# oviniciuscesar/Pseudo-Quadrature-Mirror-Filter

Hardware: NVIDIA B200
Metric: PQMF analyze+inverse throughput (n_band=16) (higher is better)
Workload: dtype f32

## Files before the change

pseudo-quadrature-mirror-filter_b200/csrc/experiments/trace_h4.cu:

```cuda
#define PQMF_H4_TRACE 1
#include <cstdio>
#include <vector>
#include "../hankel4.cuh"
using namespace pqmf;
int main(int argc, char** argv) {
  const bool pair = argc > 4 && atoi(argv[4]) != 0;
  const int B = 64; const long T = 1 << 20, F = T / 16;
  float *x, *y; uint16_t* bank; long long* tr;
  cudaMalloc(&x, (size_t)B * T * 4); cudaMalloc(&y, (size_t)B * T * 4); cudaMalloc(&bank, 2 * 27 * 4096); cudaMalloc(&tr, (64 * 64 + 512) * 8);
  cudaMemset(x, 0, (size_t)B * T * 4); cudaMemset(bank, 0, 2 * 27 * 4096); cudaMemset(tr, 0, 64 * 64 * 8);
  if (argc > 1) {
    std::vector<float> hx(1 << 22), hk(16 * 512);
    srand(3);
    for (auto& v : hx) v = (float)rand() / RAND_MAX - 0.5f;
    for (auto& v : hk) v = ((float)rand() / RAND_MAX - 0.5f) * 0.05f;
    for (size_t o = 0; o < (size_t)B * T; o += hx.size()) cudaMemcpy(x + o, hx.data(), hx.size() * 4, cudaMemcpyHostToDevice);
    std::vector<uint16_t> ia(27 * 2048), is(27 * 2048);
    hankel4_build_banks(hk.data(), 16, 512, 64, 384, ia.data(), is.data());
    cudaMemcpy(bank, ia.data(), ia.size() * 2, cudaMemcpyHostToDevice);
  }
  cudaEvent_t e0, e1; cudaEventCreate(&e0); cudaEventCreate(&e1);
  H4AnalysisParams p{};
  p.x = x; p.y = y; p.bank = bank; p.T = T; p.F = F; p.off = 256; p.parity = 0; p.trace = tr; p.trim_lo = p.trim_hi = argc > 3 ? atoi(argv[3]) : 0; p.g = h4_shape(16, 64, 384, pair, false);
  for (int rep = 0; rep < 3; ++rep) {
    int rc = (pair ? h4_launch_analysis<16, true>(p, B, 0) : h4_launch_analysis<16, false>(p, B, 0));
    cudaError_t e = cudaDeviceSynchronize();
    if (rc || e) { printf("launch rc=%d cuda=%s\n", rc, cudaGetErrorString(e)); return 1; }
  }
  const bool synth = argc > 2 && argv[2][0] == 's';
  H4SynthesisParams q{};
  q.s = x; q.out = y; q.bank = bank; q.F = F; q.o = 16; q.parity = 0; q.trace = tr; q.trim_lo = q.trim_hi = argc > 3 ? atoi(argv[3]) : 0; q.g = h4_shape(16, 64, 384, pair, true);
  if (synth) {
    cudaMemset(tr, 0, 64 * 64 * 8);
    (pair ? h4_launch_synthesis<16, true>(q, B, 0) : h4_launch_synthesis<16, false>(q, B, 0));
    cudaError_t e = cudaDeviceSynchronize();
    if (e) { printf("synthesis cuda=%s\n", cudaGetErrorString(e)); return 1; }
  }
  cudaEventRecord(e0);
  for (int rep = 0; rep < 20; ++rep) { if (synth) (pair ? h4_launch_synthesis<16, true>(q, B, 0) : h4_launch_synthesis<16, false>(q, B, 0)); else (pair ? h4_launch_analysis<16, true>(p, B, 0) : h4_launch_analysis<16, false>(p, B, 0)); }
  cudaEventRecord(e1); cudaDeviceSynchronize();
  float ms = 0; cudaEventElapsedTime(&ms, e0, e1);
  printf("%s %s data: %.1f us per launch (20 back to back)\n", synth ? "synthesis" : "analysis", argc > 1 ? "random" : "zero", ms * 50.f);
  std::vector<long long> h(64 * 64 + 512);
  cudaMemcpy(h.data(), tr, h.size() * 8, cudaMemcpyDeviceToHost);
  {
    long long cmin = 1LL << 60, cmax = 0, nmin = 1LL << 60, nmax = 0;
    for (int i = 0; i < 148; ++i) {
      const long long c = h[64 * 64 + 2 * i], n = h[64 * 64 + 2 * i + 1];
      cmin = c < cmin ? c : cmin; cmax = c > cmax ? c : cmax; nmin = n < nmin ? n : nmin; nmax = n > nmax ? n : nmax;
    }
    printf("per-CTA lifetime: %lld..%lld cycles, %lld..%lld ns -> SM clock %.0f MHz (CTA 0: %lld cycles / %lld ns)\n", cmin, cmax, nmin, nmax,
           1e3 * (double)cmax / (double)nmax, h[64 * 64], h[64 * 64 + 1]);
  }
  const long long t00 = h[(0 * 8 + 1) * 8 + 0];
  printf("warp 1 (MMA warp) and warp 5; cycles relative to the first stamp\n");
  printf("it |  start   conv   loads+publish  wait+drain(it-lag) | period\n");
  long long prev = t00;
  for (int it = 0; it < 56; ++it) {
    for (int w : {1, 5}) {
      long long* r = &h[((size_t)it * 8 + w) * 8];
      if (!r[0]) continue;
      printf("%2d w%d %8lld %6lld %6lld %10lld", it, w, r[0] - t00, r[1] - r[0], r[2] - r[1], r[5] - r[2]);
      if (w == 1) { printf(" | %lld", r[0] - prev); prev = r[0]; }
      printf("\n");
    }
    if (it == 12) it = 40;
  }
  return 0;
}
```

pseudo-quadrature-mirror-filter_b200/csrc/hankel4.cuh:

```cuda
#pragma once
#include <cuda_fp16.h>
#include <cuda_runtime.h>
#include <math.h>
#include <stdint.h>
#include <string.h>

#include <atomic>

#include "half_io.cuh"
#include "hankel16.cuh"
#include "pcm.cuh"
#include "ptx.cuh"

namespace pqmf {

constexpr int kH4Workers = 256;
constexpr int kH4Threads = kH4Workers + 32;
constexpr int kH4SynWorkers = 288;
constexpr int kH4SynThreads = kH4SynWorkers + 32;
constexpr int kH4Rows = 128;
constexpr int kH4TileSamples = 64 * kH4Rows;
constexpr int kH4MaxPlaneRows = 144;
constexpr float kH4Res = 2048.0f;

__device__ __forceinline__ uint64_t umma_desc_sw128(uint32_t smem_addr) {
  uint64_t d = 0;
  d |= (uint64_t)((smem_addr & 0x3FFFFu) >> 4);
  d |= (uint64_t)1 << 16;
  d |= (uint64_t)(1024u >> 4) << 32;
  d |= (uint64_t)1 << 46;
  d |= (uint64_t)2 << 61;
  return d;
}
__device__ __forceinline__ uint32_t sw128_offset(uint32_t byte_lin) { return byte_lin ^ (((byte_lin >> 7) & 7u) << 4); }

struct H4Shape {
  int jlo, kt, ks;
  int rows, plane;
  int bank;
  int bytes;
};
inline H4Shape h4_shape(int M, int jlo, int kt, bool pair, bool synthesis, int extra_pad_bytes = 0) {
  H4Shape g;
  g.jlo = jlo;
  g.kt = kt;
  g.ks = (kt + 64 - M + 15) / 16;
  const int pad_bytes = (synthesis ? 3 * 2 * M : 0) + extra_pad_bytes;
  g.rows = kH4Rows + (32 * g.ks + pad_bytes - 1) / 128;
  g.plane = ((g.rows * 128 + 1023) / 1024) * 1024;
  g.bank = g.ks * 2 * (pair ? 96 : 128) * 16;
  g.bytes = g.bank + 4 * g.plane + 128;
  return g;
}
inline bool h4_shape_fits(const H4Shape& g) { return g.rows <= kH4MaxPlaneRows && g.bytes <= 227 * 1024; }

template <bool PAIR>
__device__ __forceinline__ void h4_issue_mmas(uint32_t d_tmem, uint32_t plane1_addr, uint32_t plane2_addr, uint32_t bank_addr, int ks,
                                              int pad_bytes, int tlo, int thi) {
  constexpr uint32_t kBankRows = PAIR ? 96 : 128;
  const uint64_t da1 = umma_desc_sw128(plane1_addr), da2 = umma_desc_sw128(plane2_addr);
  const uint64_t db = ptx::umma_desc(bank_addr, kBankRows * 16, 128);
  const uint64_t db64 = PAIR ? ptx::umma_desc(bank_addr + 64 * 16, kBankRows * 16, 128) : db;
  constexpr uint32_t m = PAIR ? 256 : 128;
  constexpr uint32_t idesc128 = ptx::umma_idesc_f16(m, 128), idesc64 = ptx::umma_idesc_f16(m, 64);
  constexpr uint32_t kStep = 2 * kBankRows;
  auto a_step = [&](int s) {
    const uint32_t byte = 32u * (uint32_t)s + (uint32_t)pad_bytes;
    return (uint64_t)(8u * (byte >> 7) + ((byte >> 4) & 7u));
  };
  auto mma = [&](uint32_t d, uint64_t a, uint64_t bdesc, uint32_t idesc, bool acc) {
    if constexpr (PAIR) ptx::umma_pair_f16(d, a, bdesc, idesc, acc);
    else ptx::umma_f16(d, a, bdesc, idesc, acc);
  };
  for (int s = tlo; s < ks - thi; ++s) mma(d_tmem, da1 + a_step(s), db + (uint64_t)(kStep * s), idesc128, s != tlo);
  for (int s = 0; s < tlo; ++s) mma(d_tmem, da1 + a_step(s), db64 + (uint64_t)(kStep * s), idesc64, true);
  for (int s = ks - thi; s < ks; ++s) mma(d_tmem, da1 + a_step(s), db64 + (uint64_t)(kStep * s), idesc64, true);
  for (int s = tlo; s < ks - thi; ++s) mma(d_tmem + 64u, da2 + a_step(s), db64 + (uint64_t)(kStep * s), idesc64, true);
}

__device__ __forceinline__ void split2_f16s(float a, float b, uint32_t& h1_bits, uint32_t& h2_bits) {
  const __half2 h1 = __floats2half2_rn(a, b);
  const float2 h1f = __half22float2(h1);
  const float2 r = __ffma2_rn(h1f, make_float2(-kH4Res, -kH4Res), __fmul2_rn(make_float2(a, b), make_float2(kH4Res, kH4Res)));
  const __half2 h2 = __floats2half2_rn(r.x, r.y);
  h1_bits = *reinterpret_cast<const uint32_t*>(&h1);
  h2_bits = *reinterpret_cast<const uint32_t*>(&h2);
}
__device__ __forceinline__ float2 h4_combine2(uint32_t d0a, uint32_t d0b, uint32_t d1a, uint32_t d1b) {
  const float2 t = __ffma2_rn(make_float2(__uint_as_float(d1a), __uint_as_float(d1b)), make_float2(1.0f / kH4Res, 1.0f / kH4Res),
                              make_float2(__uint_as_float(d0a), __uint_as_float(d0b)));
  constexpr float kInv = 1.0f / (float)(1 << kH16ScaleLog2);
  return __fmul2_rn(t, make_float2(kInv, kInv));
}

template <int N>
__device__ __forceinline__ void h4_tmem_ld(uint32_t taddr, uint32_t (&r)[N]) {
  static_assert(N == 2 || N == 4 || N == 8 || N == 16 || N == 32, "columns per load");
  if constexpr (N == 2) ptx::tmem_ld2(taddr, r);
  else if constexpr (N == 4) ptx::tmem_ld4(taddr, r);
  else if constexpr (N == 8) ptx::tmem_ld8(taddr, r);
  else if constexpr (N == 16) ptx::tmem_ld16(taddr, r);
  else ptx::tmem_ld32(taddr, r);
}

#ifdef PQMF_H4_TRACE
#define H4_STAMP(k) do { if (blockIdx.x == 0 && (tid & 31) == 0 && it < 64) p.trace[((size_t)it * 8 + warp) * 8 + (k)] = clock64(); } while (0)
#else
#define H4_STAMP(k) do { } while (0)
#endif

struct H4Smem {
  unsigned char *bank, *planes;
  uint64_t *pfull, *mma_bar, *bankfull;
  uint32_t* tmem_slot;
};
__device__ __forceinline__ H4Smem h4_carve(unsigned char* smem, const H4Shape& g) {
  H4Smem s;
  s.bank = smem;
  s.planes = smem + g.bank;
  s.pfull = reinterpret_cast<uint64_t*>(smem + g.bank + 4 * g.plane);
  s.mma_bar = s.pfull + 2;
  s.bankfull = s.mma_bar + 2;
  s.tmem_slot = reinterpret_cast<uint32_t*>(s.bankfull + 1);
  return s;
}

template <bool PAIR>
__device__ __forceinline__ uint32_t h4_prologue(const H4Smem& s, const H4Shape& g, const uint16_t* bank_images, uint32_t rank, int worker_warps,
                                                int tid) {
  const int warp = tid >> 5;
  ptx::grid_dep_launch();
  if (tid == 0) {
    for (int i = 0; i < 2; ++i) {
      ptx::mbar_init(&s.pfull[i], worker_warps * (PAIR ? 2 : 1));
      ptx::mbar_init(&s.mma_bar[i], 1);
    }
    ptx::mbar_init(s.bankfull, 1);
    ptx::fence_barrier_init();
    ptx::mbar_arrive_expect_tx(s.bankfull, (uint32_t)g.bank);
    ptx::bulk_g2s(s.bank, reinterpret_cast<const unsigned char*>(bank_images) + (size_t)rank * g.bank, (uint32_t)g.bank, s.bankfull);
  }
  if (warp == 0) {
    if constexpr (PAIR) {
      ptx::tmem_alloc_pair(s.tmem_slot, 256);
    } else {
      ptx::tmem_alloc(s.tmem_slot, 256);
      ptx::tmem_relinquish();
    }
  }
  ptx::tc_fence_before();
  __syncthreads();
  if constexpr (PAIR) ptx::cluster_sync_all();
  ptx::tc_fence_after();
  ptx::grid_dep_wait();
  return *s.tmem_slot;
}

template <bool PAIR>
__device__ __forceinline__ void h4_teardown(uint32_t tmem, int warp) {
  ptx::tc_fence_before();
  __syncthreads();
  if constexpr (PAIR) {
    ptx::cluster_sync_all();
    if (warp == 0) ptx::tmem_dealloc_pair(tmem, 256);
  } else {
    if (warp == 0) ptx::tmem_dealloc(tmem, 256);
  }
}

template <bool PAIR>
__device__ __forceinline__ void h4_issuer_loop(const H4Smem& s, const H4Shape& g, uint32_t tmem, unsigned n_iter, int pad_bytes, int tlo,
                                               int thi, unsigned it0 = 0) {
  const uint32_t bank_addr = ptx::smem_u32(s.bank), plane_addr = ptx::smem_u32(s.planes);
  for (unsigned it = it0; it < it0 + n_iter; ++it) {
    const int pb = (int)(it & 1);
    ptx::mbar_wait(&s.pfull[pb], (it >> 1) & 1);
    ptx::tc_fence_after();
    if (ptx::elect_one_sync()) {
      h4_issue_mmas<PAIR>(tmem + (uint32_t)(pb * 128), plane_addr + (2 * pb) * g.plane, plane_addr + (2 * pb + 1) * g.plane, bank_addr, g.ks,
                          pad_bytes, tlo, thi);
      if constexpr (PAIR) ptx::umma_pair_commit(&s.mma_bar[pb]);
      else ptx::umma_commit(&s.mma_bar[pb]);
    }
    __syncwarp();
  }
}

template <bool PAIR>
__device__ __forceinline__ void h4_publish(const H4Smem& s, uint32_t pfull_leader, unsigned it, int pb, int tid, unsigned it0 = 0, unsigned bank_phase = 0) {
  ptx::fence_proxy_async();
  ptx::tc_fence_before();
  __syncwarp();
  if ((tid & 31) == 0) {
    if (it == it0) ptx::mbar_wait(s.bankfull, bank_phase & 1);
    if constexpr (PAIR) ptx::mbar_arrive_cluster(pfull_leader + 8u * pb);
    else ptx::mbar_arrive(&s.pfull[pb]);
  }
}

struct H4AnalysisParams {
  const float* x;
  PcmIn in;
  float* y;
  const uint16_t* bank;
  long T, F;
  int off;
  int parity;
  int trim_lo, trim_hi;
  int accumulate;
  int keep_in_l2;
  H4Shape g;
  long tiles_per_row, n_tiles;
#ifdef PQMF_H4_TRACE
  long long* trace;
#endif
};

template <int M, bool PAIR, H4Io IO>
__global__ void __launch_bounds__(kH4Threads, 1) h4_analysis_kernel(H4AnalysisParams p) {
  constexpr bool PCM = IO == H4Io::PCM, HALF = h4_io_half(IO);
  constexpr int FR = 64 / M;
  constexpr int HB = M / 2;
  constexpr int NO = (kH4MaxPlaneRows * 8 + kH4Workers - 1) / kH4Workers;
  extern __shared__ __align__(1024) unsigned char h4_smem[];
  const H4Shape g = p.g;
  const H4Smem sm = h4_carve(h4_smem, g);
  const int tid = threadIdx.x, warp = tid >> 5;
  constexpr int kMmaWarp = kH4Workers / 32;
  const uint32_t rank = PAIR ? ptx::cluster_ctarank() : 0u;
  const uint32_t tmem = h4_prologue<PAIR>(sm, g, p.bank, rank, kH4Workers / 32, tid);
  const uint32_t pfull_leader = PAIR ? ptx::mapa_shared(ptx::smem_u32(sm.pfull), 0) : 0u;

  const unsigned tpr = (unsigned)p.tiles_per_row;
  const unsigned step_b = gridDim.x / tpr, step_c = gridDim.x % tpr;
  unsigned b = blockIdx.x / tpr, c = blockIdx.x % tpr;
  const unsigned first_tile = PAIR ? (blockIdx.x & ~1u) : blockIdx.x;
  const unsigned n_iter = (unsigned)((p.n_tiles - first_tile + gridDim.x - 1) / gridDim.x);
  const unsigned n_rows = (unsigned)(p.n_tiles / p.tiles_per_row);
#ifdef PQMF_H4_TRACE
  long long cta_c0 = clock64(), cta_t0;
  asm volatile("mov.u64 %0, %%globaltimer;" : "=l"(cta_t0));
#endif

  if (warp == kMmaWarp) {
    if (rank == 0) h4_issuer_loop<PAIR>(sm, g, tmem, n_iter, 0, p.trim_lo, p.trim_hi);
  } else {
    const int n_octs = g.rows * 8;
    float x0[NO][8];
    auto load_window = [&](unsigned bb, unsigned cc) {
      const long s0 = (long)cc * kH4TileSamples + g.jlo - p.off;
      const float* xrow = p.x + (size_t)bb * p.T;
      const uint16_t* xhrow = reinterpret_cast<const uint16_t*>(p.x) + (size_t)bb * p.T;
#pragma unroll
      for (int r = 0; r < NO; ++r) {
        const int o = tid + kH4Workers * r;
        const long s = s0 + 8L * o;
        if (bb < n_rows && o < n_octs && s >= 0 && s < p.T) {
          if constexpr (PCM) {
            pcm_load8_raw(p.in, bb, s, p.T, x0[r]);
          } else if constexpr (HALF) {
            const float4 raw = ptx::ldg128_na(reinterpret_cast<const float4*>(xhrow + s));
            x0[r][0] = raw.x; x0[r][1] = raw.y; x0[r][2] = raw.z; x0[r][3] = raw.w;
          } else {
            ptx::ldg256_na(xrow + s, x0[r]);
          }
        } else {
#pragma unroll
          for (int e = 0; e < 8; ++e) x0[r][e] = 0.f;
        }
      }
    };
    auto convert = [&](int pb, unsigned bb, unsigned cc) {
      unsigned char* p1 = sm.planes + (2 * pb) * g.plane;
      unsigned char* p2 = p1 + g.plane;
#pragma unroll
      for (int r = 0; r < NO; ++r) {
        const int o = tid + kH4Workers * r;
        if (o < n_octs) {
          if constexpr (PCM) {
            const long s = (long)cc * kH4TileSamples + g.jlo - p.off + 8L * o;
            if (bb < n_rows && s >= 0 && s < p.T) pcm_convert8(p.in, bb, x0[r]);
          }
          if constexpr (HALF) h4_widen8<IO>(x0[r]);
          uint4 a, bq;
          split2_f16s(x0[r][0], x0[r][1], a.x, bq.x);
          split2_f16s(x0[r][2], x0[r][3], a.y, bq.y);
          split2_f16s(x0[r][4], x0[r][5], a.z, bq.z);
          split2_f16s(x0[r][6], x0[r][7], a.w, bq.w);
          const uint32_t off = sw128_offset((uint32_t)o * 16u);
          *reinterpret_cast<uint4*>(p1 + off) = a;
          *reinterpret_cast<uint4*>(p2 + off) = bq;
        }
      }
    };
    auto advance = [&](unsigned& bb, unsigned& cc) {
      bb += step_b;
      cc += step_c;
      if (cc >= tpr) {
        cc -= tpr;
        ++bb;
      }
    };
    auto epilogue = [&](unsigned bb, unsigned cc, int dbuf) {
      const int i = tid & 127, hb = tid >> 7;
      const uint32_t taddr = tmem + ((uint32_t)((warp & 3) * 32) << 16) + (uint32_t)(dbuf * 128 + HB * hb);
      const long n = ((long)cc * kH4Rows + i) * FR;
      uint32_t r0[FR][HB], r1[FR][HB];
#pragma unroll
      for (int dl = 0; dl < FR; ++dl) {
        h4_tmem_ld<HB>(taddr + dl * M, r0[dl]);
        h4_tmem_ld<HB>(taddr + 64 + dl * M, r1[dl]);
      }
      ptx::tmem_ld_wait();
      float v[FR][HB];
#pragma unroll
      for (int dl = 0; dl < FR; ++dl) {
        const uint32_t flip = (((FR > 1 ? dl : (int)(n & 1)) + p.parity) & 1) == 0 ? 0x80000000u : 0u;
#pragma unroll
        for (int kk = 0; kk < HB; kk += 2) {
          const float2 t = h4_combine2(r0[dl][kk], r0[dl][kk + 1], r1[dl][kk], r1[dl][kk + 1]);
          v[dl][kk] = t.x;
          v[dl][kk + 1] = __uint_as_float(__float_as_uint(t.y) ^ flip);
        }
      }
      if constexpr (HALF) {
        uint16_t* yp = reinterpret_cast<uint16_t*>(p.y) + ((size_t)bb * M + HB * hb) * p.F + n;
        if (n + FR - 1 < p.F && (p.F % (FR >= 8 ? 8 : FR)) == 0) {
#pragma unroll
          for (int kk = 0; kk < HB; ++kk) {
            uint16_t* q = yp + (size_t)kk * p.F;
            if constexpr (FR >= 8) {
#pragma unroll
              for (int d8 = 0; d8 < FR; d8 += 8) {
                const uint4 w = make_uint4(h4_narrow2<IO>(v[d8][kk], v[d8 + 1][kk]), h4_narrow2<IO>(v[d8 + 2][kk], v[d8 + 3][kk]),
                                           h4_narrow2<IO>(v[d8 + 4][kk], v[d8 + 5][kk]), h4_narrow2<IO>(v[d8 + 6][kk], v[d8 + 7][kk]));
                if (p.keep_in_l2) *reinterpret_cast<uint4*>(q + d8) = w;
                else __stcs(reinterpret_cast<uint4*>(q + d8), w);
              }
            } else if constexpr (FR == 4) {
              const uint2 w = make_uint2(h4_narrow2<IO>(v[0][kk], v[1][kk]), h4_narrow2<IO>(v[2][kk], v[3][kk]));
              if (p.keep_in_l2) *reinterpret_cast<uint2*>(q) = w;
              else __stcs(reinterpret_cast<uint2*>(q), w);
            } else if constexpr (FR == 2) {
              __stcs(reinterpret_cast<unsigned int*>(q), h4_narrow2<IO>(v[0][kk], v[1][kk]));
            } else {
              __stcs(reinterpret_cast<unsigned short*>(q), h4_narrow1<IO>(v[0][kk]));
            }
          }
        } else {
#pragma unroll
          for (int kk = 0; kk < HB; ++kk)
#pragma unroll
            for (int dl = 0; dl < FR; ++dl)
              if (n + dl < p.F) yp[(size_t)kk * p.F + dl] = h4_narrow1<IO>(v[dl][kk]);
        }
        return;
      }
      float* yp = p.y + ((size_t)bb * M + HB * hb) * p.F + n;
      if (n + FR - 1 < p.F && (p.F % (FR >= 4 ? 4 : FR)) == 0) {
        if (p.accumulate) {
          float prev[FR][HB];
#pragma unroll
          for (int kk = 0; kk < HB; ++kk)
#pragma unroll
            for (int dl = 0; dl < FR; ++dl) prev[dl][kk] = __ldcs(yp + (size_t)kk * p.F + dl);
#pragma unroll
          for (int kk = 0; kk < HB; ++kk)
#pragma unroll
            for (int dl = 0; dl < FR; ++dl) v[dl][kk] += prev[dl][kk];
        }
#pragma unroll
        for (int kk = 0; kk < HB; ++kk) {
          float* q = yp + (size_t)kk * p.F;
          if constexpr (FR >= 4) {
#pragma unroll
            for (int d4 = 0; d4 < FR; d4 += 4) {
              const float4 w = make_float4(v[d4][kk], v[d4 + 1][kk], v[d4 + 2][kk], v[d4 + 3][kk]);
              if (p.keep_in_l2) *reinterpret_cast<float4*>(q + d4) = w;
              else __stcs(reinterpret_cast<float4*>(q + d4), w);
            }
          } else if constexpr (FR == 2) {
            __stcs(reinterpret_cast<float2*>(q), make_float2(v[0][kk], v[1][kk]));
          } else {
            __stcs(q, v[0][kk]);
          }
        }
      } else {
#pragma unroll
        for (int kk = 0; kk < HB; ++kk)
#pragma unroll
          for (int dl = 0; dl < FR; ++dl)
            if (n + dl < p.F) yp[(size_t)kk * p.F + dl] = v[dl][kk] + (p.accumulate ? yp[(size_t)kk * p.F + dl] : 0.f);
      }
    };

    unsigned b1 = b, c1 = c;
    advance(b1, c1);
    load_window(b, c);
    unsigned prev_b = 0, prev_c = 0;
    for (unsigned it = 0; it < n_iter; ++it) {
      const int pb = (int)(it & 1);
      H4_STAMP(0);
      convert(pb, b, c);
      H4_STAMP(1);
      h4_publish<PAIR>(sm, pfull_leader, it, pb, tid);
      if (it + 1 < n_iter) load_window(b1, c1);
      H4_STAMP(2);
      if (it > 0) {
        ptx::mbar_wait(&sm.mma_bar[(it - 1) & 1], ((it - 1) >> 1) & 1);
        ptx::tc_fence_after();
        if (prev_b < n_rows) epilogue(prev_b, prev_c, (int)((it - 1) & 1));
      }
      H4_STAMP(5);
      prev_b = b;
      prev_c = c;
      b = b1;
      c = c1;
      advance(b1, c1);
    }
    ptx::mbar_wait(&sm.mma_bar[(n_iter - 1) & 1], ((n_iter - 1) >> 1) & 1);
    ptx::tc_fence_after();
    if (prev_b < n_rows) epilogue(prev_b, prev_c, (int)((n_iter - 1) & 1));
  }
#ifdef PQMF_H4_TRACE
  __syncthreads();
  if (tid == 0) {
    long long t1;
    asm volatile("mov.u64 %0, %%globaltimer;" : "=l"(t1));
    p.trace[64 * 64 + 2 * blockIdx.x] = clock64() - cta_c0;
    p.trace[64 * 64 + 2 * blockIdx.x + 1] = t1 - cta_t0;
  }
#endif
  h4_teardown<PAIR>(tmem, warp);
}

struct H4SynthesisParams {
  const float* s;
  float* out;
  int16_t* pcm_out;
  int C;
  int duo;
  const uint16_t* bank;
  long F;
  int o;
  int parity;
  int trim_lo, trim_hi;
  int accumulate;
  int reverse;
  H4Shape g;
  long tiles_per_row, n_tiles;
#ifdef PQMF_H4_TRACE
  long long* trace;
#endif
};

template <int M, bool PAIR, H4Io IO>
__global__ void __launch_bounds__(kH4SynThreads, 1) h4_synthesis_kernel(H4SynthesisParams p) {
  constexpr bool PCM = IO == H4Io::PCM, HALF = h4_io_half(IO);
  constexpr int FR = 64 / M;
  constexpr int NBG = M >= 8 ? M / 8 : 1;
  constexpr int FPI = M >= 8 ? 4 : 32 / M;
  extern __shared__ __align__(1024) unsigned char h4s_smem[];
  const H4Shape g = p.g;
  const H4Smem sm = h4_carve(h4s_smem, g);
  const int tid = threadIdx.x, warp = tid >> 5;
  constexpr int kMmaWarp = kH4SynWorkers / 32;
  const uint32_t rank = PAIR ? ptx::cluster_ctarank() : 0u;
  const uint32_t tmem = h4_prologue<PAIR>(sm, g, p.bank, rank, kH4SynWorkers / 32, tid);
  const uint32_t pfull_leader = PAIR ? ptx::mapa_shared(ptx::smem_u32(sm.pfull), 0) : 0u;

  const unsigned tpr = (unsigned)p.tiles_per_row;
  const unsigned step_b = gridDim.x / tpr, step_c = gridDim.x % tpr;
  unsigned b = blockIdx.x / tpr, c = blockIdx.x % tpr;
  const unsigned first_tile = PAIR ? (blockIdx.x & ~1u) : blockIdx.x;
  const unsigned G = (PCM && p.duo) ? 2u : 1u;
  const unsigned n_iter = G * (unsigned)((p.n_tiles - first_tile + gridDim.x - 1) / gridDim.x);
  const unsigned n_rows = (unsigned)(p.n_tiles / p.tiles_per_row);

  const int ehi = (g.jlo + g.kt) / M - 1;
  const int pad = (p.o - ehi) & 3;
  const int nbase = p.o - ehi - pad;
  if (warp == kMmaWarp) {
    if (rank == 0) h4_issuer_loop<PAIR>(sm, g, tmem, n_iter, 2 * M * pad, p.trim_lo, p.trim_hi);
  } else {
    const int n_fq = (g.rows * FR + FPI - 1) / FPI;
    const int bg = tid / n_fq, fq = tid - bg * n_fq;
    const bool has_item = tid < n_fq * NBG;
    float4 v0[8];
    auto load4h = [&](const uint16_t* at, bool ok) {
      if (!ok) return make_float4(0.f, 0.f, 0.f, 0.f);
      const float2 raw = ptx::ldg64_na(at);
      return make_float4(raw.x, raw.y, 0.f, 0.f);
    };
    auto load_frames = [&](float4 (&v)[8], unsigned bb, unsigned cc, unsigned hh) {
      if (p.reverse && bb < n_rows) {
        bb = n_rows - 1 - bb;
        cc = tpr - 1 - cc;
      }
      const long n = (long)cc * (kH4Rows * FR) + nbase + FPI * fq;
      const bool live = bb < n_rows && has_item;
      const size_t row = (size_t)bb * G + hh;
      if constexpr (HALF) {
        if constexpr (M >= 8) {
          const uint16_t* sp = reinterpret_cast<const uint16_t*>(p.s) + (row * M + 8 * bg) * p.F + n;
          const bool ok = live && n >= 0 && n + 3 < p.F;
#pragma unroll
          for (int kk = 0; kk < 8; ++kk) v[kk] = load4h(sp + (size_t)kk * p.F, ok);
        } else {
          const uint16_t* sp = reinterpret_cast<const uint16_t*>(p.s) + row * M * p.F + n;
#pragma unroll
          for (int kk = 0; kk < 8; ++kk) {
            const int b4 = kk >> 1, h = kk & 1;
            v[kk] = load4h(sp + (size_t)b4 * p.F + 4 * h, live && n + 4 * h >= 0 && n + 4 * h + 3 < p.F);
          }
        }
      } else if constexpr (M >= 8) {
        const float* sp = p.s + (row * M + 8 * bg) * p.F + n;
        const bool ok = live && n >= 0 && n + 3 < p.F;
#pragma unroll
        for (int kk = 0; kk < 8; ++kk) v[kk] = ok ? ptx::ldg128_na(reinterpret_cast<const float4*>(sp + (size_t)kk * p.F)) : make_float4(0.f, 0.f, 0.f, 0.f);
      } else {
        const float* sp = p.s + row * M * p.F + n;
#pragma unroll
        for (int kk = 0; kk < 8; ++kk) {
          const int b4 = kk >> 1, h = kk & 1;
          const bool ok = live && n + 4 * h >= 0 && n + 4 * h + 3 < p.F;
          v[kk] = ok ? ptx::ldg128_na(reinterpret_cast<const float4*>(sp + (size_t)b4 * p.F + 4 * h)) : make_float4(0.f, 0.f, 0.f, 0.f);
        }
      }
    };
    const uint32_t flip_even = (p.parity & 1) ? 0u : 0x80000000u, flip_odd = flip_even ^ 0x80000000u;
    auto advance = [&](unsigned& bb, unsigned& cc) {
      bb += step_b;
      cc += step_c;
      if (cc >= tpr) {
        cc -= tpr;
        ++bb;
      }
    };
    auto convert = [&](const float4 (&v)[8], int pb) {
      if (!has_item) return;
      unsigned char* p1 = sm.planes + (2 * pb) * g.plane;
      auto comp = [](const float4& q, int c) { return c == 0 ? q.x : c == 1 ? q.y : c == 2 ? q.z : q.w; };
#pragma unroll
      for (int j = 0; j < 4; ++j) {
        float w[8];
        uint32_t o;
        if constexpr (M >= 8) {
          const uint32_t fl = (j & 1) ? flip_odd : flip_even;
#pragma unroll
          for (int kk = 0; kk < 8; ++kk) {
            const float t = comp(v[kk], j);
            w[kk] = (kk & 1) ? __uint_as_float(__float_as_uint(t) ^ fl) : t;
          }
          o = sw128_offset((uint32_t)(4 * fq + j) * (2u * M) + 16u * bg);
        } else {
#pragma unroll
          for (int kk = 0; kk < 8; ++kk) {
            const int b4 = kk & 3, odd = kk >> 2;
            const float t = comp(v[2 * b4 + (j >> 1)], 2 * (j & 1) + odd);
            w[kk] = (b4 & 1) ? __uint_as_float(__float_as_uint(t) ^ (odd ? flip_odd : flip_even)) : t;
          }
          o = sw128_offset((uint32_t)(8 * fq + 2 * j) * (2u * M));
        }
        uint4 h1, h2;
        split2_f16s(w[0], w[1], h1.x, h2.x);
        split2_f16s(w[2], w[3], h1.y, h2.y);
        split2_f16s(w[4], w[5], h1.z, h2.z);
        split2_f16s(w[6], w[7], h1.w, h2.w);
        *reinterpret_cast<uint4*>(p1 + o) = h1;
        *reinterpret_cast<uint4*>(p1 + g.plane + o) = h2;
      }
    };
    uint32_t held[4][4];
    auto epilogue = [&](unsigned bb, unsigned cc, unsigned hh, int dbuf) {
      if (p.reverse) {
        bb = n_rows - 1 - bb;
        cc = tpr - 1 - cc;
      }
      const size_t row = (size_t)bb * G + hh;
      const int i = tid & 127, hb = tid >> 7, lane = tid & 31;
      const uint32_t taddr = tmem + ((uint32_t)((warp & 3) * 32) << 16) + (uint32_t)(dbuf * 128 + 2 * hb * 16);
      uint32_t r0[2][16], r1[2][16];
      ptx::tmem_ld16(taddr, r0[0]);
      ptx::tmem_ld16(taddr + 64, r1[0]);
      ptx::tmem_ld16(taddr + 16, r0[1]);
      ptx::tmem_ld16(taddr + 80, r1[1]);
      ptx::tmem_ld_wait();
      float val[4][8];
#pragma unroll
      for (int q = 0; q < 4; ++q)
#pragma unroll
        for (int e = 0; e < 8; e += 2) {
          const int c0 = 8 * (q & 1) + e;
          const float2 t = h4_combine2(r0[q >> 1][c0], r0[q >> 1][c0 + 1], r1[q >> 1][c0], r1[q >> 1][c0 + 1]);
          val[q][e] = t.x;
          val[q][e + 1] = t.y;
        }
      const bool b0 = lane & 1, b1 = lane & 2;
#pragma unroll
      for (int pr = 0; pr < 2; ++pr)
#pragma unroll
        for (int e = 0; e < 8; ++e) {
          const float recv = __shfl_xor_sync(0xffffffffu, b0 ? val[2 * pr][e] : val[2 * pr + 1][e], 1);
          val[2 * pr + 1][e] = b0 ? val[2 * pr + 1][e] : recv;
          val[2 * pr][e] = b0 ? recv : val[2 * pr][e];
        }
#pragma unroll
      for (int u = 0; u < 2; ++u)
#pragma unroll
        for (int e = 0; e < 8; ++e) {
          const float recv = __shfl_xor_sync(0xffffffffu, b1 ? val[u][e] : val[u + 2][e], 2);
          val[u + 2][e] = b1 ? val[u + 2][e] : recv;
          val[u][e] = b1 ? recv : val[u][e];
        }
      const long total = p.F * M;
      const long t0 = (long)cc * kH4TileSamples + 64 * (i & ~3) + 32 * hb + 8 * (lane & 3);
      if constexpr (PCM) {
        if (G == 2) {
#pragma unroll
          for (int q = 0; q < 4; ++q) {
            uint32_t w[4];
#pragma unroll
            for (int k = 0; k < 4; ++k)
              w[k] = (uint32_t)(uint16_t)pcm_quantise(val[q][2 * k]) | ((uint32_t)(uint16_t)pcm_quantise(val[q][2 * k + 1]) << 16);
            if (hh == 0) {
#pragma unroll
              for (int k = 0; k < 4; ++k) held[q][k] = w[k];
            } else if (t0 + 64 * q + 7 < total) {
              float lr[8];
#pragma unroll
              for (int k = 0; k < 4; ++k) {
                lr[2 * k] = __uint_as_float(__byte_perm(held[q][k], w[k], 0x5410));
                lr[2 * k + 1] = __uint_as_float(__byte_perm(held[q][k], w[k], 0x7632));
              }
              ptx::stg256_cs(reinterpret_cast<float*>(p.pcm_out + ((size_t)bb * total + t0 + 64 * q) * 2), lr);
            }
          }
          return;
        }
#pragma unroll
        for (int q = 0; q < 4; ++q)
          if (t0 + 64 * q + 7 < total) pcm_store8(p.pcm_out, p.C, (long)row, t0 + 64 * q, total, val[q]);
        return;
      }
      if constexpr (HALF) {
        uint16_t* op = reinterpret_cast<uint16_t*>(p.out) + row * total + t0;
#pragma unroll
        for (int q = 0; q < 4; ++q)
          if (t0 + 64 * q + 7 < total) {
            const uint4 w = make_uint4(h4_narrow2<IO>(val[q][0], val[q][1]), h4_narrow2<IO>(val[q][2], val[q][3]), h4_narrow2<IO>(val[q][4], val[q][5]),
                                       h4_narrow2<IO>(val[q][6], val[q][7]));
            __stcs(reinterpret_cast<uint4*>(op + (size_t)q * 64), w);
          }
        return;
      }
      float* op = p.out + row * total + t0;
#pragma unroll
      for (int q = 0; q < 4; ++q)
        if (t0 + 64 * q + 7 < total) {
          if (p.accumulate) {
            float prev[8];
            ptx::ldg256_cs(op + (size_t)q * 64, prev);
#pragma unroll
            for (int e = 0; e < 8; ++e) val[q][e] += prev[e];
          }
          ptx::stg256_cs(op + (size_t)q * 64, val[q]);
        }
    };

    auto next_visit = [&](unsigned& bb, unsigned& cc, unsigned& hh) {
      if (++hh == G) {
        hh = 0;
        advance(bb, cc);
      }
    };
    unsigned h = 0, b1 = b, c1 = c, h1 = 0;
    next_visit(b1, c1, h1);
    load_frames(v0, b, c, h);
    unsigned prev_b = 0, prev_c = 0, prev_h = 0;
    for (unsigned it = 0; it < n_iter; ++it) {
      const int pb = (int)(it & 1);
      H4_STAMP(0);
      if constexpr (HALF) {
        float4 w[8];
#pragma unroll
        for (int kk = 0; kk < 8; ++kk) w[kk] = h4_widen4<IO>(v0[kk]);
        convert(w, pb);
      } else {
        convert(v0, pb);
      }
      H4_STAMP(1);
      h4_publish<PAIR>(sm, pfull_leader, it, pb, tid);
      if (it + 1 < n_iter) load_frames(v0, b1, c1, h1);
      H4_STAMP(2);
      if (it > 0) {
        ptx::mbar_wait(&sm.mma_bar[(it - 1) & 1], ((it - 1) >> 1) & 1);
        ptx::tc_fence_after();
        if (warp < 8 && prev_b < n_rows) epilogue(prev_b, prev_c, prev_h, (int)((it - 1) & 1));
      }
      H4_STAMP(5);
      prev_b = b;
      prev_c = c;
      prev_h = h;
      b = b1;
      c = c1;
      h = h1;
      next_visit(b1, c1, h1);
    }
    ptx::mbar_wait(&sm.mma_bar[(n_iter - 1) & 1], ((n_iter - 1) >> 1) & 1);
    ptx::tc_fence_after();
    if (warp < 8 && prev_b < n_rows) epilogue(prev_b, prev_c, prev_h, (int)((n_iter - 1) & 1));
  }
  h4_teardown<PAIR>(tmem, warp);
}

struct H4Configured {
  std::atomic<int> bytes[64];
  H4Configured() {
    for (auto& b : bytes) b.store(0, std::memory_order_relaxed);
  }
};
inline int h4_sm_count(int dev) {
  static std::atomic<int> sm_count[64];
  int n = sm_count[dev].load(std::memory_order_relaxed);
  if (n == 0) {
    cudaDeviceGetAttribute(&n, cudaDevAttrMultiProcessorCount, dev);
    n = n > 0 ? n : 148;
    sm_count[dev].store(n, std::memory_order_relaxed);
  }
  return n;
}
template <typename Kern>
inline int h4_configure(Kern kern, int bytes, H4Configured& configured, int& sm_count_out) {
  int dev = 0;
  cudaGetDevice(&dev);
  dev &= 63;
  if (configured.bytes[dev].load(std::memory_order_acquire) < bytes) {
    cudaError_t e = cudaFuncSetAttribute(kern, cudaFuncAttributeMaxDynamicSharedMemorySize, bytes);
    if (e != cudaSuccess) return (int)e;
    int seen = configured.bytes[dev].load(std::memory_order_relaxed);
    while (seen < bytes && !configured.bytes[dev].compare_exchange_weak(seen, bytes, std::memory_order_release)) {
    }
  }
  sm_count_out = h4_sm_count(dev);
  return 0;
}

template <bool PAIR, typename Kern, typename Params>
inline int h4_launch(Kern kern, Params p, int B, long row_samples, int threads, H4Configured& configured, cudaStream_t st) {
  int sms = 0;
  if (!h4_shape_fits(p.g)) return -2;
  if (int e = h4_configure(kern, p.g.bytes, configured, sms)) return e;
  p.tiles_per_row = (row_samples + kH4TileSamples - 1) / kH4TileSamples;
  p.n_tiles = p.tiles_per_row * B;
  if (p.tiles_per_row >= (1L << 31) || p.n_tiles >= (1L << 40)) return -2;
  long grid = PAIR ? (sms & ~1) : sms;
  const long want = PAIR ? ((p.n_tiles + 1) & ~1L) : p.n_tiles;
  if (grid > want) grid = want;
  if constexpr (PAIR) {
    cudaLaunchConfig_t cfg = {};
    cfg.gridDim = dim3((unsigned)grid);
    cfg.blockDim = dim3((unsigned)threads);
    cfg.dynamicSmemBytes = (size_t)p.g.bytes;
    cfg.stream = st;
    cudaLaunchAttribute attr[2];
    attr[0].id = cudaLaunchAttributeClusterDimension;
    attr[0].val.clusterDim.x = 2;
    attr[0].val.clusterDim.y = 1;
    attr[0].val.clusterDim.z = 1;
    attr[1].id = cudaLaunchAttributeProgrammaticStreamSerialization;
    attr[1].val.programmaticStreamSerializationAllowed = 1;
    cfg.attrs = attr;
    cfg.numAttrs = 2;
    return (int)cudaLaunchKernelEx(&cfg, kern, p);
  } else {
    kern<<<(unsigned)grid, threads, p.g.bytes, st>>>(p);
    return (int)cudaGetLastError();
  }
}

template <int M, bool PAIR>
int h4_launch_analysis(H4AnalysisParams p, int B, cudaStream_t st, H4Io io = H4Io::F32) {
  static H4Configured configured[4];
  if (p.in.pcm != nullptr) io = H4Io::PCM;
  if (io != H4Io::F32) {
    if constexpr (PAIR) {
      switch (io) {
        case H4Io::PCM: return h4_launch<PAIR>(h4_analysis_kernel<M, PAIR, H4Io::PCM>, p, B, p.F * M, kH4Threads, configured[1], st);
        case H4Io::F16: return h4_launch<PAIR>(h4_analysis_kernel<M, PAIR, H4Io::F16>, p, B, p.F * M, kH4Threads, configured[2], st);
        case H4Io::BF16: return h4_launch<PAIR>(h4_analysis_kernel<M, PAIR, H4Io::BF16>, p, B, p.F * M, kH4Threads, configured[3], st);
        default: return -2;
      }
    } else {
      return -2;
    }
  }
  return h4_launch<PAIR>(h4_analysis_kernel<M, PAIR, H4Io::F32>, p, B, p.F * M, kH4Threads, configured[0], st);
}

template <int M, bool PAIR>
int h4_launch_synthesis(H4SynthesisParams p, int B, cudaStream_t st, H4Io io = H4Io::F32) {
  static H4Configured configured[4];
  if (p.pcm_out != nullptr) {
    if constexpr (PAIR) {
      p.duo = (p.C == 2 && B % 2 == 0) ? 1 : 0;
      return h4_launch<PAIR>(h4_synthesis_kernel<M, PAIR, H4Io::PCM>, p, p.duo ? B / 2 : B, p.F * M, kH4SynThreads, configured[1], st);
    } else {
      return -2;
    }
  }
  if (h4_io_half(io)) {
    if constexpr (PAIR) {
      if (io == H4Io::F16) return h4_launch<PAIR>(h4_synthesis_kernel<M, PAIR, H4Io::F16>, p, B, p.F * M, kH4SynThreads, configured[2], st);
      return h4_launch<PAIR>(h4_synthesis_kernel<M, PAIR, H4Io::BF16>, p, B, p.F * M, kH4SynThreads, configured[3], st);
    } else {
      return -2;
    }
  }
  return h4_launch<PAIR>(h4_synthesis_kernel<M, PAIR, H4Io::F32>, p, B, p.F * M, kH4SynThreads, configured[0], st);
}

inline void hankel4_build_banks(const float* hk , int M, int L, int jlo, int kt, uint16_t* img_analysis, uint16_t* img_synthesis) {
  auto bits = [](float v) {
    const __half h = __float2half_rn(v);
    uint16_t u;
    memcpy(&u, &h, 2);
    return u;
  };
  const int ks = (kt + 64 - M + 15) / 16, kp = 16 * ks;
  const int elo = jlo / M, ehi = (jlo + kt) / M - 1;
  const float sa = (float)(1 << kH16ScaleLog2), ss = (float)M * sa;
  for (int kc = 0; kc < kp / 8; ++kc)
    for (int row = 0; row < 128; ++row)
      for (int e8 = 0; e8 < 8; ++e8) {
        const int kap = 8 * kc + e8;
        const int part = row / 64, delta = (row % 64) / M, q = row % M;
        const size_t at = ((size_t)kc * 128 + row) * 8 + e8;
        {
          const int j = kap - M * delta;
          const float v = (j >= 0 && j < kt && jlo + j < L) ? sa * hk[(size_t)q * L + jlo + j] : 0.f;
          const float c1 = __half2float(__float2half_rn(v));
          img_analysis[at] = part == 0 ? bits(c1) : bits((v - c1) * kH4Res);
        }
        {
          const int e = kap / M, kb = kap % M, lag = delta + ehi - e;
          const float v = (lag >= elo && lag <= ehi && M * lag + q < L) ? ss * hk[(size_t)kb * L + M * lag + q] : 0.f;
          const float c1 = __half2float(__float2half_rn(v));
          img_synthesis[at] = part == 0 ? bits(c1) : bits((v - c1) * kH4Res);
        }
      }
}

inline void hankel4_pair_image(const uint16_t* single , int ks, uint16_t* pair ) {
  const int chunks = 2 * ks;
  for (int r = 0; r < 2; ++r)
    for (int kc = 0; kc < chunks; ++kc)
      for (int row = 0; row < 96; ++row) {
        const int src = row < 64 ? 64 * r + row : 32 * r + (row - 64);
        memcpy(pair + (((size_t)r * chunks + kc) * 96 + row) * 8, single + ((size_t)kc * 128 + src) * 8, 16);
      }
}

inline int hankel4_pick_trim(const float* hk , int M, int L, int jlo, int kt, bool synthesis, double budget, int max_trim = 7) {
  const int ks = (kt + 64 - M + 15) / 16, fr = 64 / M, elo = jlo / M, ehi = (jlo + kt) / M - 1;
  int best = 0;
  for (int trim = 1; trim <= max_trim && ks - 2 * trim >= 1; ++trim) {
    double worst = 0.0;
    for (int delta = 0; delta < fr; ++delta)
      for (int q = 0; q < M; ++q) {
        double sum = 0.0;
        for (int side = 0; side < 2; ++side)
          for (int t = 0; t < trim; ++t) {
            const int s = side ? ks - 1 - t : t;
            for (int e16 = 0; e16 < 16; ++e16) {
              const int kap = 16 * s + e16;
              if (!synthesis) {
                const int j = kap - M * delta;
                if (j >= 0 && j < kt && jlo + j < L) sum += fabs((double)hk[(size_t)q * L + jlo + j]);
              } else {
                const int e = kap / M, kb = kap % M, lag = delta + ehi - e;
                if (lag >= elo && lag <= ehi && M * lag + q < L) sum += (double)M * fabs((double)hk[(size_t)kb * L + M * lag + q]);
              }
            }
          }
        worst = sum > worst ? sum : worst;
      }
    if (2.0 * worst / 2048.0 <= budget) best = trim;
    else break;
  }
  return best;
}

}
```

Measured before the change: 259,700.

## Split epilogue drain into dedicated warps with TMEM accumulator free barriers

New measurement: 198,500 (median of 6 runs). 0.764x the previous value.

```diff
diff --git a/pseudo-quadrature-mirror-filter_b200/csrc/experiments/trace_h4.cu b/pseudo-quadrature-mirror-filter_b200/csrc/experiments/trace_h4.cu
--- a/pseudo-quadrature-mirror-filter_b200/csrc/experiments/trace_h4.cu
+++ b/pseudo-quadrature-mirror-filter_b200/csrc/experiments/trace_h4.cu
@@ -53,14 +53,15 @@
            1e3 * (double)cmax / (double)nmax, h[64 * 64], h[64 * 64 + 1]);
   }
   const long long t00 = h[(0 * 8 + 1) * 8 + 0];
-  printf("warp 1 (MMA warp) and warp 5; cycles relative to the first stamp\n");
-  printf("it |  start   conv   loads+publish  wait+drain(it-lag) | period\n");
+  printf("converter warps 1, 5 and drain warps 1, 5 (slot = warp within its role); cycles relative to the first stamp\n");
+  printf("it    |  conv: start  wait+conv  loads+publish | drain: start  wait(mma)  drain+release | conv period\n");
   long long prev = t00;
   for (int it = 0; it < 56; ++it) {
     for (int w : {1, 5}) {
       long long* r = &h[((size_t)it * 8 + w) * 8];
       if (!r[0]) continue;
-      printf("%2d w%d %8lld %6lld %6lld %10lld", it, w, r[0] - t00, r[1] - r[0], r[2] - r[1], r[5] - r[2]);
+      printf("%2d s%d  | %12lld %10lld %14lld | %12lld %10lld %14lld", it, w, r[0] - t00, r[1] - r[0], r[2] - r[1], r[3] - t00, r[4] - r[3],
+             r[5] - r[4]);
       if (w == 1) { printf(" | %lld", r[0] - prev); prev = r[0]; }
       printf("\n");
     }
diff --git a/pseudo-quadrature-mirror-filter_b200/csrc/hankel4.cuh b/pseudo-quadrature-mirror-filter_b200/csrc/hankel4.cuh
--- a/pseudo-quadrature-mirror-filter_b200/csrc/hankel4.cuh
+++ b/pseudo-quadrature-mirror-filter_b200/csrc/hankel4.cuh
@@ -18,6 +18,9 @@
 constexpr int kH4Threads = kH4Workers + 32;
 constexpr int kH4SynWorkers = 288;
 constexpr int kH4SynThreads = kH4SynWorkers + 32;
+constexpr int kH4Drainers = 256;
+constexpr int kH4OffThreads = kH4Workers + kH4Drainers + 32;
+constexpr int kH4SynOffThreads = kH4SynWorkers + kH4Drainers + 32;
 constexpr int kH4Rows = 128;
 constexpr int kH4TileSamples = 64 * kH4Rows;
 constexpr int kH4MaxPlaneRows = 144;
@@ -104,15 +107,16 @@
 }
 
 #ifdef PQMF_H4_TRACE
-#define H4_STAMP(k) do { if (blockIdx.x == 0 && (tid & 31) == 0 && it < 64) p.trace[((size_t)it * 8 + warp) * 8 + (k)] = clock64(); } while (0)
+#define H4_STAMP(w, k) do { if (blockIdx.x == 0 && (tid & 31) == 0 && it < 64 && (w) < 8) p.trace[((size_t)it * 8 + (w)) * 8 + (k)] = clock64(); } while (0)
 #else
-#define H4_STAMP(k) do { } while (0)
+#define H4_STAMP(w, k) do { } while (0)
 #endif
 
 struct H4Smem {
   unsigned char *bank, *planes;
   uint64_t *pfull, *mma_bar, *bankfull;
   uint32_t* tmem_slot;
+  uint64_t* dfree;
 };
 __device__ __forceinline__ H4Smem h4_carve(unsigned char* smem, const H4Shape& g) {
   H4Smem s;
@@ -122,7 +126,13 @@
   s.mma_bar = s.pfull + 2;
   s.bankfull = s.mma_bar + 2;
   s.tmem_slot = reinterpret_cast<uint32_t*>(s.bankfull + 1);
+  s.dfree = s.bankfull + 2;
   return s;
+}
+template <bool PAIR>
+__device__ __forceinline__ void h4_init_dfree(const H4Smem& s, int tid) {
+  if (tid == 0)
+    for (int i = 0; i < 2; ++i) ptx::mbar_init(&s.dfree[i], (kH4Drainers / 32) * (PAIR ? 2 : 1));
 }
 
 template <bool PAIR>
@@ -168,13 +178,16 @@
   }
 }
 
-template <bool PAIR>
+template <bool PAIR, bool DFREE = false>
 __device__ __forceinline__ void h4_issuer_loop(const H4Smem& s, const H4Shape& g, uint32_t tmem, unsigned n_iter, int pad_bytes, int tlo,
                                                int thi, unsigned it0 = 0) {
   const uint32_t bank_addr = ptx::smem_u32(s.bank), plane_addr = ptx::smem_u32(s.planes);
   for (unsigned it = it0; it < it0 + n_iter; ++it) {
     const int pb = (int)(it & 1);
     ptx::mbar_wait(&s.pfull[pb], (it >> 1) & 1);
+    if constexpr (DFREE) {
+      if (it >= it0 + 2) ptx::mbar_wait(&s.dfree[pb], ((it - 2) >> 1) & 1);
+    }
     ptx::tc_fence_after();
     if (ptx::elect_one_sync()) {
       h4_issue_mmas<PAIR>(tmem + (uint32_t)(pb * 128), plane_addr + (2 * pb) * g.plane, plane_addr + (2 * pb + 1) * g.plane, bank_addr, g.ks,
@@ -195,6 +208,16 @@
     if (it == it0) ptx::mbar_wait(s.bankfull, bank_phase & 1);
     if constexpr (PAIR) ptx::mbar_arrive_cluster(pfull_leader + 8u * pb);
     else ptx::mbar_arrive(&s.pfull[pb]);
+  }
+}
+
+template <bool PAIR>
+__device__ __forceinline__ void h4_release_acc(const H4Smem& s, uint32_t dfree_leader, int pb, int tid) {
+  ptx::tc_fence_before();
+  __syncwarp();
+  if ((tid & 31) == 0) {
+    if constexpr (PAIR) ptx::mbar_arrive_cluster(dfree_leader + 8u * pb);
+    else ptx::mbar_arrive(&s.dfree[pb]);
   }
 }
 
@@ -217,7 +240,7 @@
 };
 
 template <int M, bool PAIR, H4Io IO>
-__global__ void __launch_bounds__(kH4Threads, 1) h4_analysis_kernel(H4AnalysisParams p) {
+__global__ void __launch_bounds__(kH4OffThreads, 1) h4_analysis_kernel(H4AnalysisParams p) {
   constexpr bool PCM = IO == H4Io::PCM, HALF = h4_io_half(IO);
   constexpr int FR = 64 / M;
   constexpr int HB = M / 2;
@@ -226,10 +249,12 @@
   const H4Shape g = p.g;
   const H4Smem sm = h4_carve(h4_smem, g);
   const int tid = threadIdx.x, warp = tid >> 5;
-  constexpr int kMmaWarp = kH4Workers / 32;
+  constexpr int kDrain0 = kH4Workers / 32, kMmaWarp = (kH4Workers + kH4Drainers) / 32;
   const uint32_t rank = PAIR ? ptx::cluster_ctarank() : 0u;
+  h4_init_dfree<PAIR>(sm, tid);
   const uint32_t tmem = h4_prologue<PAIR>(sm, g, p.bank, rank, kH4Workers / 32, tid);
   const uint32_t pfull_leader = PAIR ? ptx::mapa_shared(ptx::smem_u32(sm.pfull), 0) : 0u;
+  const uint32_t dfree_leader = PAIR ? ptx::mapa_shared(ptx::smem_u32(sm.dfree), 0) : 0u;
 
   const unsigned tpr = (unsigned)p.tiles_per_row;
   const unsigned step_b = gridDim.x / tpr, step_c = gridDim.x % tpr;
@@ -243,16 +268,15 @@
 #endif
 
   if (warp == kMmaWarp) {
-    if (rank == 0) h4_issuer_loop<PAIR>(sm, g, tmem, n_iter, 0, p.trim_lo, p.trim_hi);
+    if (rank == 0) h4_issuer_loop<PAIR, true>(sm, g, tmem, n_iter, 0, p.trim_lo, p.trim_hi);
   } else {
     const int n_octs = g.rows * 8;
     float x0[NO][8];
-    auto load_window = [&](unsigned bb, unsigned cc) {
+    auto load_window = [&](unsigned bb, unsigned cc, int r) {
       const long s0 = (long)cc * kH4TileSamples + g.jlo - p.off;
       const float* xrow = p.x + (size_t)bb * p.T;
       const uint16_t* xhrow = reinterpret_cast<const uint16_t*>(p.x) + (size_t)bb * p.T;
-#pragma unroll
-      for (int r = 0; r < NO; ++r) {
+      {
         const int o = tid + kH4Workers * r;
         const long s = s0 + 8L * o;
         if (bb < n_rows && o < n_octs && s >= 0 && s < p.T) {
@@ -270,11 +294,10 @@
         }
       }
     };
-    auto convert = [&](int pb, unsigned bb, unsigned cc) {
+    auto convert = [&](int pb, unsigned bb, unsigned cc, int r) {
       unsigned char* p1 = sm.planes + (2 * pb) * g.plane;
       unsigned char* p2 = p1 + g.plane;
-#pragma unroll
-      for (int r = 0; r < NO; ++r) {
+      {
         const int o = tid + kH4Workers * r;
         if (o < n_octs) {
           if constexpr (PCM) {
@@ -302,7 +325,7 @@
       }
     };
     auto epilogue = [&](unsigned bb, unsigned cc, int dbuf) {
-      const int i = tid & 127, hb = tid >> 7;
+      const int i = tid & 127, hb = (warp - kDrain0) >> 2;
       const uint32_t taddr = tmem + ((uint32_t)((warp & 3) * 32) << 16) + (uint32_t)(dbuf * 128 + HB * hb);
       const long n = ((long)cc * kH4Rows + i) * FR;
       uint32_t r0[FR][HB], r1[FR][HB];
@@ -394,33 +417,43 @@
       }
     };
 
-    unsigned b1 = b, c1 = c;
-    advance(b1, c1);
-    load_window(b, c);
-    unsigned prev_b = 0, prev_c = 0;
-    for (unsigned it = 0; it < n_iter; ++it) {
-      const int pb = (int)(it & 1);
-      H4_STAMP(0);
-      convert(pb, b, c);
-      H4_STAMP(1);
-      h4_publish<PAIR>(sm, pfull_leader, it, pb, tid);
-      if (it + 1 < n_iter) load_window(b1, c1);
-      H4_STAMP(2);
-      if (it > 0) {
-        ptx::mbar_wait(&sm.mma_bar[(it - 1) & 1], ((it - 1) >> 1) & 1);
+    if (warp < kDrain0) {
+      unsigned b1 = b, c1 = c;
+      advance(b1, c1);
+#pragma unroll
+      for (int r = 0; r < NO; ++r) load_window(b, c, r);
+      for (unsigned it = 0; it < n_iter; ++it) {
+        const int pb = (int)(it & 1);
+        H4_STAMP(warp, 0);
+        if (it >= 2) {
+          ptx::mbar_wait(&sm.mma_bar[pb], ((it - 2) >> 1) & 1);
+          ptx::tc_fence_after();
+        }
+#pragma unroll
+        for (int r = 0; r < NO; ++r) {
+          convert(pb, b, c, r);
+          if (it + 1 < n_iter) load_window(b1, c1, r);
+        }
+        H4_STAMP(warp, 1);
+        h4_publish<PAIR>(sm, pfull_leader, it, pb, tid);
+        H4_STAMP(warp, 2);
+        b = b1;
+        c = c1;
+        advance(b1, c1);
+      }
+    } else {
+      for (unsigned it = 0; it < n_iter; ++it) {
+        const int pb = (int)(it & 1);
+        H4_STAMP(warp - kDrain0, 3);
+        ptx::mbar_wait(&sm.mma_bar[pb], (it >> 1) & 1);
         ptx::tc_fence_after();
-        if (prev_b < n_rows) epilogue(prev_b, prev_c, (int)((it - 1) & 1));
-      }
-      H4_STAMP(5);
-      prev_b = b;
-      prev_c = c;
-      b = b1;
-      c = c1;
-      advance(b1, c1);
+        H4_STAMP(warp - kDrain0, 4);
+        if (b < n_rows) epilogue(b, c, pb);
+        h4_release_acc<PAIR>(sm, dfree_leader, pb, tid);
+        H4_STAMP(warp - kDrain0, 5);
+        advance(b, c);
+      }
     }
-    ptx::mbar_wait(&sm.mma_bar[(n_iter - 1) & 1], ((n_iter - 1) >> 1) & 1);
-    ptx::tc_fence_after();
-    if (prev_b < n_rows) epilogue(prev_b, prev_c, (int)((n_iter - 1) & 1));
   }
 #ifdef PQMF_H4_TRACE
   __syncthreads();
@@ -455,7 +488,7 @@
 };
 
 template <int M, bool PAIR, H4Io IO>
-__global__ void __launch_bounds__(kH4SynThreads, 1) h4_synthesis_kernel(H4SynthesisParams p) {
+__global__ void __launch_bounds__(kH4SynOffThreads, 1) h4_synthesis_kernel(H4SynthesisParams p) {
   constexpr bool PCM = IO == H4Io::PCM, HALF = h4_io_half(IO);
   constexpr int FR = 64 / M;
   constexpr int NBG = M >= 8 ? M / 8 : 1;
@@ -464,13 +497,15 @@
   const H4Shape g = p.g;
   const H4Smem sm = h4_carve(h4s_smem, g);
   const int tid = threadIdx.x, warp = tid >> 5;
-  constexpr int kMmaWarp = kH4SynWorkers / 32;
+  constexpr int kDrain0 = kH4SynWorkers / 32, kMmaWarp = (kH4SynWorkers + kH4Drainers) / 32;
   const uint32_t rank = PAIR ? ptx::cluster_ctarank() : 0u;
+  h4_init_dfree<PAIR>(sm, tid);
   const uint32_t tmem = h4_prologue<PAIR>(sm, g, p.bank, rank, kH4SynWorkers / 32, tid);
   const uint32_t pfull_leader = PAIR ? ptx::mapa_shared(ptx::smem_u32(sm.pfull), 0) : 0u;
+  const uint32_t dfree_leader = PAIR ? ptx::mapa_shared(ptx::smem_u32(sm.dfree), 0) : 0u;
 
   const unsigned tpr = (unsigned)p.tiles_per_row;
-  const unsigned step_b = gridDim.x / tpr, step_c = gridDim.x % tpr;
+  const unsigned step_b = gridDim.x / tpr;
   unsigned b = blockIdx.x / tpr, c = blockIdx.x % tpr;
   const unsigned first_tile = PAIR ? (blockIdx.x & ~1u) : blockIdx.x;
   const unsigned G = (PCM && p.duo) ? 2u : 1u;
@@ -481,7 +516,7 @@
   const int pad = (p.o - ehi) & 3;
   const int nbase = p.o - ehi - pad;
   if (warp == kMmaWarp) {
-    if (rank == 0) h4_issuer_loop<PAIR>(sm, g, tmem, n_iter, 2 * M * pad, p.trim_lo, p.trim_hi);
+    if (rank == 0) h4_issuer_loop<PAIR, true>(sm, g, tmem, n_iter, 2 * M * pad, p.trim_lo, p.trim_hi);
   } else {
     const int n_fq = (g.rows * FR + FPI - 1) / FPI;
     const int bg = tid / n_fq, fq = tid - bg * n_fq;
@@ -532,7 +567,7 @@
     const uint32_t flip_even = (p.parity & 1) ? 0u : 0x80000000u, flip_odd = flip_even ^ 0x80000000u;
     auto advance = [&](unsigned& bb, unsigned& cc) {
       bb += step_b;
-      cc += step_c;
+      cc += gridDim.x - step_b * tpr;
       if (cc >= tpr) {
         cc -= tpr;
         ++bb;
@@ -579,7 +614,7 @@
         cc = tpr - 1 - cc;
       }
       const size_t row = (size_t)bb * G + hh;
-      const int i = tid & 127, hb = tid >> 7, lane = tid & 31;
+      const int i = tid & 127, hb = (warp - kDrain0) >> 2, lane = tid & 31;
       const uint32_t taddr = tmem + ((uint32_t)((warp & 3) * 32) << 16) + (uint32_t)(dbuf * 128 + 2 * hb * 16);
       uint32_t r0[2][16], r1[2][16];
       ptx::tmem_ld16(taddr, r0[0]);
@@ -675,42 +710,48 @@
         advance(bb, cc);
       }
     };
-    unsigned h = 0, b1 = b, c1 = c, h1 = 0;
-    next_visit(b1, c1, h1);
-    load_frames(v0, b, c, h);
-    unsigned prev_b = 0, prev_c = 0, prev_h = 0;
-    for (unsigned it = 0; it < n_iter; ++it) {
-      const int pb = (int)(it & 1);
-      H4_STAMP(0);
-      if constexpr (HALF) {
-        float4 w[8];
-#pragma unroll
-        for (int kk = 0; kk < 8; ++kk) w[kk] = h4_widen4<IO>(v0[kk]);
-        convert(w, pb);
-      } else {
-        convert(v0, pb);
-      }
-      H4_STAMP(1);
-      h4_publish<PAIR>(sm, pfull_leader, it, pb, tid);
-      if (it + 1 < n_iter) load_frames(v0, b1, c1, h1);
-      H4_STAMP(2);
-      if (it > 0) {
-        ptx::mbar_wait(&sm.mma_bar[(it - 1) & 1], ((it - 1) >> 1) & 1);
+    unsigned h = 0;
+    if (warp < kDrain0) {
+      unsigned b1 = b, c1 = c, h1 = 0;
+      next_visit(b1, c1, h1);
+      load_frames(v0, b, c, h);
+      for (unsigned it = 0; it < n_iter; ++it) {
+        const int pb = (int)(it & 1);
+        H4_STAMP(warp, 0);
+        if (it >= 2) {
+          ptx::mbar_wait(&sm.mma_bar[pb], ((it - 2) >> 1) & 1);
+          ptx::tc_fence_after();
+        }
+        if constexpr (HALF) {
+          float4 w[8];
+#pragma unroll
+          for (int kk = 0; kk < 8; ++kk) w[kk] = h4_widen4<IO>(v0[kk]);
+          convert(w, pb);
+        } else {
+          convert(v0, pb);
+        }
+        if (it + 1 < n_iter) load_frames(v0, b1, c1, h1);
+        H4_STAMP(warp, 1);
+        h4_publish<PAIR>(sm, pfull_leader, it, pb, tid);
+        H4_STAMP(warp, 2);
+        b = b1;
+        c = c1;
+        h = h1;
+        next_visit(b1, c1, h1);
+      }
+    } else {
+      for (unsigned it = 0; it < n_iter; ++it) {
+        const int pb = (int)(it & 1);
+        H4_STAMP(warp - kDrain0, 3);
+        ptx::mbar_wait(&sm.mma_bar[pb], (it >> 1) & 1);
         ptx::tc_fence_after();
-        if (warp < 8 && prev_b < n_rows) epilogue(prev_b, prev_c, prev_h, (int)((it - 1) & 1));
-      }
-      H4_STAMP(5);
-      prev_b = b;
-      prev_c = c;
-      prev_h = h;
-      b = b1;
-      c = c1;
-      h = h1;
-      next_visit(b1, c1, h1);
+        H4_STAMP(warp - kDrain0, 4);
+        if (b < n_rows) epilogue(b, c, h, pb);
+        h4_release_acc<PAIR>(sm, dfree_leader, pb, tid);
+        H4_STAMP(warp - kDrain0, 5);
+        next_visit(b, c, h);
+      }
     }
-    ptx::mbar_wait(&sm.mma_bar[(n_iter - 1) & 1], ((n_iter - 1) >> 1) & 1);
-    ptx::tc_fence_after();
-    if (warp < 8 && prev_b < n_rows) epilogue(prev_b, prev_c, prev_h, (int)((n_iter - 1) & 1));
   }
   h4_teardown<PAIR>(tmem, warp);
 }
@@ -787,16 +828,16 @@
   if (io != H4Io::F32) {
     if constexpr (PAIR) {
       switch (io) {
-        case H4Io::PCM: return h4_launch<PAIR>(h4_analysis_kernel<M, PAIR, H4Io::PCM>, p, B, p.F * M, kH4Threads, configured[1], st);
-        case H4Io::F16: return h4_launch<PAIR>(h4_analysis_kernel<M, PAIR, H4Io::F16>, p, B, p.F * M, kH4Threads, configured[2], st);
-        case H4Io::BF16: return h4_launch<PAIR>(h4_analysis_kernel<M, PAIR, H4Io::BF16>, p, B, p.F * M, kH4Threads, configured[3], st);
+        case H4Io::PCM: return h4_launch<PAIR>(h4_analysis_kernel<M, PAIR, H4Io::PCM>, p, B, p.F * M, kH4OffThreads, configured[1], st);
+        case H4Io::F16: return h4_launch<PAIR>(h4_analysis_kernel<M, PAIR, H4Io::F16>, p, B, p.F * M, kH4OffThreads, configured[2], st);
+        case H4Io::BF16: return h4_launch<PAIR>(h4_analysis_kernel<M, PAIR, H4Io::BF16>, p, B, p.F * M, kH4OffThreads, configured[3], st);
         default: return -2;
       }
     } else {
       return -2;
     }
   }
-  return h4_launch<PAIR>(h4_analysis_kernel<M, PAIR, H4Io::F32>, p, B, p.F * M, kH4Threads, configured[0], st);
+  return h4_launch<PAIR>(h4_analysis_kernel<M, PAIR, H4Io::F32>, p, B, p.F * M, kH4OffThreads, configured[0], st);
 }
 
 template <int M, bool PAIR>
@@ -805,20 +846,20 @@
   if (p.pcm_out != nullptr) {
     if constexpr (PAIR) {
       p.duo = (p.C == 2 && B % 2 == 0) ? 1 : 0;
-      return h4_launch<PAIR>(h4_synthesis_kernel<M, PAIR, H4Io::PCM>, p, p.duo ? B / 2 : B, p.F * M, kH4SynThreads, configured[1], st);
+      return h4_launch<PAIR>(h4_synthesis_kernel<M, PAIR, H4Io::PCM>, p, p.duo ? B / 2 : B, p.F * M, kH4SynOffThreads, configured[1], st);
     } else {
       return -2;
     }
   }
   if (h4_io_half(io)) {
     if constexpr (PAIR) {
-      if (io == H4Io::F16) return h4_launch<PAIR>(h4_synthesis_kernel<M, PAIR, H4Io::F16>, p, B, p.F * M, kH4SynThreads, configured[2], st);
-      return h4_launch<PAIR>(h4_synthesis_kernel<M, PAIR, H4Io::BF16>, p, B, p.F * M, kH4SynThreads, configured[3], st);
+      if (io == H4Io::F16) return h4_launch<PAIR>(h4_synthesis_kernel<M, PAIR, H4Io::F16>, p, B, p.F * M, kH4SynOffThreads, configured[2], st);
+      return h4_launch<PAIR>(h4_synthesis_kernel<M, PAIR, H4Io::BF16>, p, B, p.F * M, kH4SynOffThreads, configured[3], st);
     } else {
       return -2;
     }
   }
-  return h4_launch<PAIR>(h4_synthesis_kernel<M, PAIR, H4Io::F32>, p, B, p.F * M, kH4SynThreads, configured[0], st);
+  return h4_launch<PAIR>(h4_synthesis_kernel<M, PAIR, H4Io::F32>, p, B, p.F * M, kH4SynOffThreads, configured[0], st);
 }
 
 inline void hankel4_build_banks(const float* hk , int M, int L, int jlo, int kt, uint16_t* img_analysis, uint16_t* img_synthesis) {
```
